# j-min/HiREST

Measured on AMD Instinct MI355X. Metric: encoded frames/sec (EVA-CLIP-g/14 224^2), higher is better.
Workload: dtype bf16

## Files before the change

hirest_amd/csrc/gemm.hip:

```cpp
#include <cstdio>
#include <atomic>
#include "gemm_shared.h"

namespace {


constexpr int BM = 128, BN = 128, BK = 64;
constexpr int STAGE_BYTES = (BM + BN) * BK * 2;

template <int EPI>
__device__ __forceinline__ void epilogue_store(const GemmP& p, int m, int n, f32x4 v) {
    if (p.bias) {
        f32x4 b = *reinterpret_cast<const f32x4*>(p.bias + n);
        v += b;
    }
    if constexpr (EPI == HIREST_EPI_BIAS_BF16 || EPI == HIREST_EPI_BIAS_GELU_BF16 || EPI == HIREST_EPI_BIAS_QGELU_BF16) {
        if constexpr (EPI == HIREST_EPI_BIAS_GELU_BF16) {
#pragma unroll
            for (int i = 0; i < 4; ++i) v[i] = gelu_erf(v[i]);
        }
        if constexpr (EPI == HIREST_EPI_BIAS_QGELU_BF16) {
#pragma unroll
            for (int i = 0; i < 4; ++i) v[i] = quick_gelu(v[i]);
        }
// ... 1000 lines not shown
    const int np_solo = team_walk && solo ? (np * solo + nslot / 2) / nslot : 0, np_team = np - np_solo;
    int count;
    if (!team_walk) count = (nunit - slot + nslot - 1) / nslot;
    else if (slot < tslots) { const int tm = slot / p.nbn; count = tm < np_team ? (np_team - tm + teams - 1) / teams : 0; }
    else { const int sl_ = slot - tslots; count = sl_ < np_solo ? ((np_solo - sl_ + solo - 1) / solo) * p.nbn : 0; }
    if (count <= 0) return;
    if (stagger) {
        const int who = stagger == 1 ? (slot & 3) : stagger == 2 ? (xcd & 3) : ((slot + xcd) & 7);
        const int units = who * (stagger == 3 ? (p.K / Q_BK + 15) / 16 : (p.K / Q_BK + 7) / 8);
        for (int i = 0; i < units; ++i) __builtin_amdgcn_s_sleep(127);
    }
    auto team_origin = [&](int i, int& M0, int& N0) {
        if (p.rev) i = count - 1 - i;
        int panel, col;
        if (slot < tslots) { panel = slot / p.nbn + i * teams; col = slot % p.nbn; }
        else { panel = np_team + (slot - tslots) + (i / p.nbn) * solo; col = i % p.nbn; }
        M0 = (p_lo + panel) * T_BM; N0 = col * T_BN;
    };
    auto tile_origin = [&](int j, int& M0, int& N0) {
        if (team_walk) { team_origin((j - slot) / nslot, M0, N0); return; }
        if (p.rev) j = nunit - 1 - j;
        if (panel_major) {
            const int mt_i = j / p.nbn;
            M0 = (p_lo + mt_i) * T_BM; N0 = (j - mt_i * p.nbn) * T_BN;
            return;
        }
        const int g_ = j / (GROUP_M * p.nbn);
        const int r = j - g_ * GROUP_M * p.nbn;
        int gcount = np - g_ * GROUP_M; gcount = gcount > GROUP_M ? GROUP_M : gcount;
        const int nt_i = r / gcount, mt_i = p_lo + g_ * GROUP_M + (r - nt_i * gcount);
        M0 = mt_i * T_BM; N0 = nt_i * T_BN;
    };

    const int nst = p.K / Q_BK;
    uint32_t a_off[2][2], w_off[2][2];
    int a_lds[2][2], w_lds[2][2];
    const char* a_base; const char* w_base;
#pragma unroll
    for (int hsel = 0; hsel < 2; ++hsel)
#pragma unroll
        for (int q = 0; q < 2; ++q) {
            const int j = 2 * wave + q;
            a_lds[hsel][q] = ((j >> 3) * 128 + hsel * 64 + (j & 7) * 8) * 128;
            w_lds[hsel][q] = Q_WOFF + ((j >> 2) * 64 + hsel * 32 + (j & 3) * 8) * 128;
        }
    auto set_sources = [&](int M0, int N0) {
#pragma unroll
        for (int hsel = 0; hsel < 2; ++hsel)
#pragma unroll
            for (int q = 0; q < 2; ++q) {
                const int ra0 = (a_lds[hsel][q] >> 7) + (lane >> 3);
                const int rw0 = ((w_lds[hsel][q] - Q_WOFF) >> 7) + (lane >> 3);
                const int ca = (lane & 7) ^ ((ra0 >> 1) & 7), cw = (lane & 7) ^ ((rw0 >> 1) & 7);
                int ra = p.M - 1 - M0; ra = ra0 < ra ? ra0 : ra;
                int rn = p.N - 1 - N0; rn = rw0 < rn ? rw0 : rn;
                a_off[hsel][q] = (uint32_t)(ra * (int)p.lda + ca * 8) * 2u;
                w_off[hsel][q] = (uint32_t)(rn * (int)p.ldw + cw * 8) * 2u;
            }
        const int Ma = (DBG && (sched & 8)) ? (p_lo + ((M0 / T_BM - p_lo) & 3)) * T_BM : M0;
        a_base = reinterpret_cast<const char*>(p.A + (int64_t)Ma * p.lda);
        w_base = reinterpret_cast<const char*>(p.W + (int64_t)N0 * p.ldw);
    };
    int dma_j = slot, dma_k = 0, dma_g = 0;
    bool dma_live = true;
    const char* a1_base; uint32_t a1_off[2]; int a1_k = 0, a1_g = 0;
    auto issue_a0 = [&]() {
        char* buf = smem + (dma_g & 1) * Q_STEP;
        const char* ab = a_base + (int64_t)dma_k * (Q_BK * 2);
        glds16(ab + a_off[0][0], buf + a_lds[0][0]);
        glds16(ab + a_off[0][1], buf + a_lds[0][1]);
    };
    auto issue_w = [&](int hsel) {
        char* buf = smem + (dma_g & 1) * Q_STEP;
        const char* wb = w_base + (int64_t)dma_k * (Q_BK * 2);
        glds16(wb + w_off[hsel][0], buf + w_lds[hsel][0]);
        glds16(wb + w_off[hsel][1], buf + w_lds[hsel][1]);
    };
    auto issue_a1_pending = [&]() {
        char* buf = smem + (a1_g & 1) * Q_STEP;
        const char* ab = a1_base + (int64_t)a1_k * (Q_BK * 2);
        glds16(ab + a1_off[0], buf + a_lds[1][0]);
        glds16(ab + a1_off[1], buf + a_lds[1][1]);
    };
    auto advance = [&]() {
        a1_base = a_base; a1_off[0] = a_off[1][0]; a1_off[1] = a_off[1][1]; a1_k = dma_k; a1_g = dma_g;
        ++dma_g;
        if (dma_live && ++dma_k == nst) {
            dma_j += nslot;
            if (dma_j < slot + count * nslot) { int m0, n0; tile_origin(dma_j, m0, n0); set_sources(m0, n0); dma_k = 0; }
            else { dma_live = false; dma_k = nst - 1; }
        }
    };

    const int frow = lane & 15, fsw = (frow >> 1) & 7, kg = lane >> 4;
    const int a_frag = (wr * 128 + frow) * (Q_BK * 2);
    const int w_frag = Q_WOFF + (wc * 64 + frow) * (Q_BK * 2);
    int koff[2];
#pragma unroll
    for (int h = 0; h < 2; ++h) koff[h] = ((4 * h + kg) ^ fsw) << 4;
    struct FA { bf16x8 v[4][2]; };
    struct FW { bf16x8 v[2][2]; };
    FA Af;
    FW W0, W1;
    auto read_a = [&](const char* buf, int a) {
#pragma unroll
        for (int m = 0; m < 4; ++m)
#pragma unroll
            for (int h = 0; h < 2; ++h) Af.v[m][h] = *reinterpret_cast<const bf16x8*>(buf + a_frag + (a * 64 + m * 16) * 128 + koff[h]);
    };
    auto read_w = [&](const char* buf, int b, FW& f) {
#pragma unroll
        for (int n = 0; n < 2; ++n)
#pragma unroll
            for (int h = 0; h < 2; ++h) f.v[n][h] = *reinterpret_cast<const bf16x8*>(buf + w_frag + (b * 32 + n * 16) * 128 + koff[h]);
    };
    f32x4 acc[8][NI];
    auto mfma_q = [&](int a, int b, FW& fw) {
        __builtin_amdgcn_s_setprio(1);
        if constexpr (X3) {
#pragma unroll
            for (int g3 = 0; g3 < 3; ++g3)
#pragma unroll
                for (int m = 0; m < 4; ++m)
#pragma unroll
                    for (int n = 0; n < 2; ++n)
                        acc[a * 4 + m][b * 2 + n] = __builtin_amdgcn_mfma_f32_16x16x32_bf16(fw.v[n][g3 == 1 ? 1 : 0], Af.v[m][g3 == 0 ? 1 : 0],
                                                                                             acc[a * 4 + m][b * 2 + n], 0, 0, 0);
        } else {
#pragma unroll
            for (int h = 0; h < 2; ++h)
#pragma unroll
                for (int m = 0; m < 4; ++m)
#pragma unroll
                    for (int n = 0; n < 2; ++n)
                        acc[a * 4 + m][b * 2 + n] = __builtin_amdgcn_mfma_f32_16x16x32_bf16(fw.v[n][h], Af.v[m][h], acc[a * 4 + m][b * 2 + n], 0, 0, 0);
        }
        __builtin_amdgcn_s_setprio(0);
    };
    auto bar = [&]() { __builtin_amdgcn_s_barrier(); };

    {
        int m0, n0;
        tile_origin(slot, m0, n0);
        set_sources(m0, n0);
    }
    for (int i = 0; i < 2; ++i) { issue_a0(); issue_w(0); issue_w(1); advance(); issue_a1_pending(); }
    bool a1_valid = false;
    HX_WAIT_VM(0);
    bar();
    if (grp == 1) bar();

    char* stg = smem + 2 * Q_STEP + wave * p_stg_bytes(EPI);
    int g = 0;
    for (int j = slot; j < slot + count * nslot; j += nslot) {
        int M0, N0;
        tile_origin(j, M0, N0);
        const bool active = (N0 + wc * 64 < p.N) && (M0 + wr * 128 < p.M);
        if (active) {
            if constexpr (epi_is_lnfold(EPI)) {
                int r0 = M0 + wr * 128 + 2 * lane;
                const int last = (p.M - 1) & ~1;
                r0 = r0 < last ? r0 : last;
                glds16(reinterpret_cast<const float*>(p.aux0) + 2 * (int64_t)r0, stg + P_STG);
                int c = N0 + wc * 64 + 4 * (lane & 15);
                c = c < p.N - 4 ? c : p.N - 4;
                const float* src = ((lane & 16) || !p.bias) ? reinterpret_cast<const float*>(p.aux1) : p.bias;
                glds16(src + c, stg + P_BCS);
            }
#pragma unroll
            for (int i = 0; i < 8; ++i)
#pragma unroll
                for (int jn = 0; jn < NI; ++jn) acc[i][jn] = f32x4{0.f, 0.f, 0.f, 0.f};
        }
        if (active && PH2) {
            for (int t = 0; t < nst; ++t, ++g) {
                const char* cur = smem + (g & 1) * Q_STEP;
                HX_WAIT_VM(6);
                __builtin_amdgcn_sched_barrier(0);
                read_a(cur, 0); read_w(cur, 0, W0); read_w(cur, 1, W1);
                if (a1_valid) issue_a1_pending();
                HX_WAIT_LGKM0();
                bar();
                mfma_q(0, 0, W0);
                mfma_q(0, 1, W1);
                bar();
                HX_WAIT_VM(2);
                __builtin_amdgcn_sched_barrier(0);
                read_a(cur, 1);
                issue_a0(); issue_w(0); issue_w(1);
                advance();
                a1_valid = true;
                HX_WAIT_LGKM0();
                bar();
                mfma_q(1, 1, W1);
                mfma_q(1, 0, W0);
                bar();
            }
            epilogue_p<EPI, NI, epi_is_lnfold(EPI), 8, RD, false, DBG, epi_is_lnfold(EPI)>(p, acc, stg, M0 + wr * 128, N0 + wc * 64, lane);
        } else if (PH2) {
            for (int t = 0; t < nst; ++t, ++g) {
                HX_WAIT_VM(6);
                if (a1_valid) issue_a1_pending();
                bar(); bar();
                HX_WAIT_VM(2);
                issue_a0(); issue_w(0); issue_w(1);
                advance();
                a1_valid = true;
                bar(); bar();
            }
        } else if (active) {
            for (int t = 0; t < nst; ++t, ++g) {
                const char* cur = smem + (g & 1) * Q_STEP;
                HX_WAIT_VM(8);
                __builtin_amdgcn_sched_barrier(0);
                read_a(cur, 0); read_w(cur, 0, W0);
                if (a1_valid) issue_a1_pending();
                bar();
                HX_WAIT_LGKM0();
                mfma_q(0, 0, W0);
                bar();
                HX_WAIT_VM(8);
                __builtin_amdgcn_sched_barrier(0);
                read_w(cur, 1, W1);
                bar();
                HX_WAIT_LGKM0();
                mfma_q(0, 1, W1);
                bar();
                __builtin_amdgcn_sched_barrier(0);
                read_a(cur, 1);
                issue_a0(); issue_w(0);
                bar();
                HX_WAIT_LGKM0();
                mfma_q(1, 1, W1);
                bar();
                HX_WAIT_VM(8);
                __builtin_amdgcn_sched_barrier(0);
                issue_w(1);
                advance();
                a1_valid = true;
                bar();
                mfma_q(1, 0, W0);
                bar();
            }
            if constexpr (epi_is_lnfold(EPI)) HX_WAIT_VM(8);
            epilogue_p<EPI, NI, epi_is_lnfold(EPI), 8, RD, false, DBG, epi_is_lnfold(EPI)>(p, acc, stg, M0 + wr * 128, N0 + wc * 64, lane);
        } else {
            for (int t = 0; t < nst; ++t, ++g) {
                HX_WAIT_VM(8);
                if (a1_valid) issue_a1_pending();
                bar(); bar();
                HX_WAIT_VM(8);
                bar(); bar();
                issue_a0(); issue_w(0);
                bar(); bar();
                HX_WAIT_VM(8);
                issue_w(1);
                advance();
                a1_valid = true;
                bar(); bar();
            }
        }
    }
    if (grp == 0) bar();
    HX_WAIT_VM(0);
}

template <int EPI, int RD = 1>
__global__ __launch_bounds__(512) void gemm_pp256(GemmP p) { pp256_body<EPI, RD, false>(p); }
template <int EPI>
__global__ __launch_bounds__(512) void gemm_pp256x3(GemmP p) { pp256_body<EPI, 1, true>(p); }
template <int EPI>
__global__ __launch_bounds__(512) void gemm_pq256(GemmP p) { pp256_body<EPI, (EPI == HIREST_EPI_BIAS_RESID2_LNSTATS ? HIREST_S2_RD : 1), false, 1>(p); }
template <int EPI>
__global__ __launch_bounds__(512) void gemm_pq256x3(GemmP p) { pp256_body<EPI, 1, true, 1>(p); }
template <int EPI>
__global__ __launch_bounds__(512) void gemm_pq256_dbg(GemmP p) { pp256_body<EPI, (EPI == HIREST_EPI_BIAS_RESID2_LNSTATS ? HIREST_S2_RD : 1), false, 1, true>(p); }



static inline void tiles256(GemmP& p) {
    p.nbm = (p.M + T_BM - 1) / T_BM; p.nbn = (p.N + T_BN - 1) / T_BN;
    p.ppx = (p.nbm + 7) / 8;
}

template <auto KERN, int LDS>
int launch_tiles(GemmP p, hipStream_t s) {
    static HirestDevCfg cfg;
    if (int e = hirest_configure(KERN, LDS, cfg)) return e;
    tiles256(p);
    hipLaunchKernelGGL(KERN, dim3(8 * p.ppx * p.nbn), dim3(512), LDS, s, p);
    return hirest_launch_status();
}
template <auto KERN, int NW, int LDS>
int launch_persistent(GemmP p, hipStream_t s) {
    static HirestDevCfg cfg;
    int cus = 0;
    if (int e = hirest_configure(KERN, LDS, cfg, &cus)) return e;
    tiles256(p);
    int nslot = cus / 8; nslot = nslot < 1 ? 1 : nslot;
    const int per_xcd = p.ppx * p.nbn;
    if (nslot > per_xcd) nslot = per_xcd;
    hipLaunchKernelGGL(KERN, dim3(8 * nslot), dim3(64 * NW), LDS, s, p);
    return hirest_launch_status();
}
constexpr int p_lds(int epi, int nw) { return 2 * Q_STEP + nw * p_stg_bytes(epi); }

template <int EPI>
int launch_t128(GemmP p, hipStream_t s) {
    hipLaunchKernelGGL(gemm_t128<EPI>, dim3(8 * p.ppx * p.nbn), dim3(256), 2 * STAGE_BYTES, s, p);
    return hirest_launch_status();
}

template <int EPI, int WM>
int launch_t128x3(GemmP p, hipStream_t s) {
    static HirestDevCfg cfg;
    auto kern = gemm_t128x3<EPI, WM>;
    constexpr int LDS = 4 * (64 * WM + BN) * BK * 2;
    if (int e = hirest_configure(kern, LDS, cfg)) return e;
    p.nbm = (p.M + 64 * WM - 1) / (64 * WM);
    p.ppx = (p.nbm + 7) / 8;
    p.flat = p.nbm < 32 ? 1 : 0;
    p.ksplit = 1;
    if (EPI == HIREST_EPI_BIAS_RESID_F32 && p.flat && p.aux0 && !p.aux1) {
        const int ntile = p.nbm * p.nbn, nk = p.K / BK;
        for (int S = 4; S >= 2; --S)
            if (nk % S == 0 && nk / S >= 8 && ntile * S <= 256) { p.ksplit = S; break; }
        p.part = reinterpret_cast<float*>(p.aux0);
    }
    const int grid = p.flat ? 8 * ((p.nbm * p.nbn * p.ksplit + 7) / 8) : 8 * p.ppx * p.nbn;
    hipLaunchKernelGGL(kern, dim3(grid), dim3(256 * WM), LDS, s, p);
    if (p.ksplit > 1) {
        const int64_t total = (int64_t)p.M * (p.N / 4);
        int blocks = (int)((total + 255) / 256); blocks = blocks > 2048 ? 2048 : blocks;
        hipLaunchKernelGGL(splitk_reduce_kernel, dim3(blocks), dim3(256), 0, s, p.part, p.ksplit, p.bias, reinterpret_cast<float*>(p.out), p.ldo, p.M, p.N);
    }
    return hirest_launch_status();
}

}
// ... 179 lines not shown
```

hirest_amd/csrc/gemm_shared.h:

```cpp
#pragma once
#include "common.h"
#include "profile.h"

namespace {

struct GemmP {
    const bf16_t* A; int64_t lda;
    const bf16_t* W; int64_t ldw;
    const float* bias;
    void* out; int64_t ldo;
    int M, N, K;
    const float* pos; int P;
    int rev;
    void* aux0; void* aux1;
    int nbm, nbn, ppx;
    int epi_dbg;
    int stagger;
    int sched;
    int dbg;
    int flat = 0;
    int ksplit = 1;
    float* part = nullptr;
};
constexpr int GEMM_DBG_IGNORE_REVERSE = 1 << 9;
constexpr int GEMM_DBG_STAGGER_SHIFT = 10, GEMM_DBG_STAGGER_MASK = 3;
constexpr int GEMM_DBG_EPI_SHIFT = 12, GEMM_DBG_EPI_MASK = 15;
constexpr int GEMM_DBG_SCHED_SHIFT = 16, GEMM_DBG_SCHED_MASK = 15;
constexpr int GEMM_DBG_PQ_SWITCHES = GEMM_DBG_STAGGER_MASK << GEMM_DBG_STAGGER_SHIFT | GEMM_DBG_EPI_MASK << GEMM_DBG_EPI_SHIFT | GEMM_DBG_SCHED_MASK << GEMM_DBG_SCHED_SHIFT;
constexpr int GEMM_DBG_KERNEL_BITS = ~(GEMM_DBG_IGNORE_REVERSE | GEMM_DBG_PQ_SWITCHES);

constexpr int GROUP_M = 8;
template <bool DBG = false>
__device__ __forceinline__ void xcd_panels(const GemmP& p, int xcd, int& p_lo, int& np) {
    if (DBG && (p.sched & 1)) { p_lo = xcd * p.ppx; np = p.nbm - p_lo; np = np > p.ppx ? p.ppx : np; return; }
    p_lo = (int)(((long long)xcd * p.nbm) >> 3);
    np = (int)(((long long)(xcd + 1) * p.nbm) >> 3) - p_lo;
}
constexpr int T_BM = 256, T_BN = 256;
#define HX_WAIT_VM(n) asm volatile("s_waitcnt vmcnt(" #n ")" ::: "memory")
#define HX_WAIT_LGKM0() asm volatile("s_waitcnt lgkmcnt(0)" ::: "memory")
constexpr int Q_BK = 64;
constexpr int Q_STEP = (T_BM + T_BN) * Q_BK * 2;
constexpr int Q_WOFF = T_BM * Q_BK * 2;

#ifndef HIREST_X3_GELU_POLY
#define HIREST_X3_GELU_POLY 1
#endif
#ifndef HIREST_S2_BUFFER_EPILOGUE
#define HIREST_S2_BUFFER_EPILOGUE 1
#endif
#ifndef HIREST_S2_RD
#define HIREST_S2_RD 2
#endif
constexpr int P_STG = 2048;
constexpr bool epi_is_lnfold(int epi) { return epi == HIREST_EPI_LNFOLD_BF16 || epi == HIREST_EPI_LNFOLD_GELU_BF16; }
constexpr int P_BCS = P_STG + 1024;
constexpr int p_stg_bytes(int epi) {
    return epi_is_lnfold(epi) ? P_STG + 2048 : (epi == HIREST_EPI_BIAS_RESID2_LNSTATS && HIREST_S2_BUFFER_EPILOGUE) ? 2 * P_STG : P_STG;
}

#define HX_LDS_ORDER() asm volatile("" ::: "memory")

__device__ __forceinline__ float dpp_xor1(float v) {
    return __builtin_bit_cast(float, __builtin_amdgcn_mov_dpp(__builtin_bit_cast(int, v), 0xB1, 0xf, 0xf, true));
}
__device__ __forceinline__ float sum8(float v) {
    v += __builtin_bit_cast(float, __builtin_amdgcn_mov_dpp(__builtin_bit_cast(int, v), 0xB1, 0xf, 0xf, true));
    v += __builtin_bit_cast(float, __builtin_amdgcn_mov_dpp(__builtin_bit_cast(int, v), 0x4E, 0xf, 0xf, true));
    v += __builtin_bit_cast(float, __builtin_amdgcn_mov_dpp(__builtin_bit_cast(int, v), 0x141, 0xf, 0xf, true));
    return v;
}
typedef __attribute__((ext_vector_type(4))) unsigned u32x4;
typedef __attribute__((ext_vector_type(2))) unsigned u32x2;
constexpr unsigned HX_OOB = 0x80000000u;
__device__ __forceinline__ __amdgpu_buffer_rsrc_t hx_rsrc(const void* base, unsigned bytes) {
    return __builtin_amdgcn_make_buffer_rsrc(const_cast<void*>(base), 0, (int)bytes, 0x00020000);
}

template <int NI, int NM, int RD, bool S2 = false, bool DBG = false>
__device__ __forceinline__ void epilogue_lnstats(const GemmP& p, f32x4 (&acc)[8][NI], int jc, char* stg, int Mw, int Nw, int lane) {
    const int epi_dbg = DBG ? p.epi_dbg : 0, sched = DBG ? p.sched : 0;
    const int srow = lane & 15, kg = lane >> 4, sw = lane & 7;
    const int rr = lane >> 3, rc = lane & 7;
    float* outp = reinterpret_cast<float*>(p.out);
    bf16_t* xb = reinterpret_cast<bf16_t*>(p.aux0);
    float* part = reinterpret_cast<float*>(p.aux1);
    const int G = (p.N + 63) >> 6;
    f32x4 bv[4];
#pragma unroll
    for (int n = 0; n < 4; ++n) {
        const int col = Nw + n * 16 + 4 * kg;
        bv[n] = (p.bias && col < p.N) ? *reinterpret_cast<const f32x4*>(p.bias + col) : f32x4{0.f, 0.f, 0.f, 0.f};
    }
    const int n0 = Nw + rc * 4, n1 = Nw + 32 + rc * 4;
    bf16_t* xlo = reinterpret_cast<bf16_t*>(p.out);
    auto load_res = [&](int mi, f32x4 (&o)[2][2]) {
#pragma unroll
        for (int it = 0; it < 2; ++it) {
            const int m = Mw + mi * 16 + it * 8 + rr;
            if constexpr (S2) {
                const int64_t mr = m < p.M ? m : p.M - 1;
                const int col = (rc & 1) ? n1 - 4 : n0;
                union { bf16x8 v; bf16x4 h[2]; float f[4]; } hv, lv;
                hv.v = bf16x8{0, 0, 0, 0, 0, 0, 0, 0}; lv.v = hv.v;
                if (col + 8 <= p.N && !(epi_dbg & 1)) {
                    if (sched & 2) {
                        hv.v = *reinterpret_cast<const bf16x8*>(xb + mr * p.N + col);
                        lv.v = *reinterpret_cast<const bf16x8*>(xlo + mr * p.ldo + col);
                    } else {
                        hv.v = __builtin_nontemporal_load(reinterpret_cast<const bf16x8*>(xb + mr * p.N + col));
                        lv.v = __builtin_nontemporal_load(reinterpret_cast<const bf16x8*>(xlo + mr * p.ldo + col));
                    }
                }
                o[0][it] = __builtin_bit_cast(f32x4, hv.v);
                o[1][it] = __builtin_bit_cast(f32x4, lv.v);
                continue;
            }
            const float* row = outp + (int64_t)(m < p.M ? m : p.M - 1) * p.ldo;
            o[0][it] = (n0 < p.N && !(epi_dbg & 1)) ? __builtin_nontemporal_load(reinterpret_cast<const f32x4*>(row + n0)) : f32x4{0.f, 0.f, 0.f, 0.f};
            o[1][it] = (n1 < p.N && !(epi_dbg & 1)) ? __builtin_nontemporal_load(reinterpret_cast<const f32x4*>(row + n1)) : f32x4{0.f, 0.f, 0.f, 0.f};
        }
    };
    f32x4 ring[RD + 1][2][2];
#pragma unroll
    for (int a = 0; a < RD && a < NM; ++a) load_res(a, ring[a]);
#pragma unroll
    for (int mi = 0; mi < NM; ++mi) {
        if (mi + RD < NM) load_res(mi + RD, ring[(mi + RD) % (RD + 1)]);
        f32x4 (&oc)[2][2] = ring[mi % (RD + 1)];
        if constexpr (S2) {
#pragma unroll
            for (int it = 0; it < 2; ++it) {
                union { bf16x8 v; bf16x4 h[2]; float f[4]; } hv, lv;
                hv.v = __builtin_bit_cast(bf16x8, oc[0][it]); lv.v = __builtin_bit_cast(bf16x8, oc[1][it]);
                union { bf16x4 v; float f[2]; } hs, hr, ls, lr;
                hs.v = (rc & 1) ? hv.h[0] : hv.h[1];
                ls.v = (rc & 1) ? lv.h[0] : lv.h[1];
                hr.f[0] = dpp_xor1(hs.f[0]); hr.f[1] = dpp_xor1(hs.f[1]);
                lr.f[0] = dpp_xor1(ls.f[0]); lr.f[1] = dpp_xor1(ls.f[1]);
                const bf16x4 h0 = (rc & 1) ? hr.v : hv.h[0], h1 = (rc & 1) ? hv.h[1] : hr.v;
                const bf16x4 l0 = (rc & 1) ? lr.v : lv.h[0], l1 = (rc & 1) ? lv.h[1] : lr.v;
#pragma unroll
                for (int e = 0; e < 4; ++e) { oc[0][it][e] = (float)h0[e] + (float)l0[e]; oc[1][it][e] = (float)h1[e] + (float)l1[e]; }
            }
        }
        f32x4 wv[2][2];
#pragma unroll
        for (int h = 0; h < 2; ++h) {
#pragma unroll
            for (int nn = 0; nn < 2; ++nn)
                *reinterpret_cast<f32x4*>(stg + srow * 128 + (((nn * 4 + kg) ^ sw) << 4)) = acc[mi][jc + h * 2 + nn] + bv[h * 2 + nn];
            HX_LDS_ORDER();
#pragma unroll
            for (int it = 0; it < 2; ++it) {
                const int r = it * 8 + rr;
                wv[h][it] = *reinterpret_cast<const f32x4*>(stg + r * 128 + ((rc ^ (r & 7)) << 4)) + oc[h][it];
            }
            HX_LDS_ORDER();
        }
#pragma unroll
        for (int it = 0; it < 2; ++it) {
            const int m = Mw + mi * 16 + it * 8 + rr;
            const bool okm = m < p.M, ok0 = okm && n0 < p.N, ok1 = okm && n1 < p.N;
            if constexpr (!S2) {
                if (ok0 && !(epi_dbg & 2)) __builtin_nontemporal_store(wv[0][it], reinterpret_cast<f32x4*>(outp + (int64_t)m * p.ldo + n0));
                if (ok1 && !(epi_dbg & 2)) __builtin_nontemporal_store(wv[1][it], reinterpret_cast<f32x4*>(outp + (int64_t)m * p.ldo + n1));
            }
            union { bf16x4 v; float f[2]; } b0, b1, snd, rcv;
            float ps = 0.f, pq = 0.f;
#pragma unroll
            for (int e = 0; e < 4; ++e) {
                b0.v[e] = (bf16_t)wv[0][it][e]; b1.v[e] = (bf16_t)wv[1][it][e];
                const float f0 = ok0 ? (float)b0.v[e] : 0.f, f1 = ok1 ? (float)b1.v[e] : 0.f;
                ps += f0 + f1; pq = fmaf(f0, f0, fmaf(f1, f1, pq));
            }
            snd.v = (rc & 1) ? b0.v : b1.v;
            rcv.f[0] = dpp_xor1(snd.f[0]); rcv.f[1] = dpp_xor1(snd.f[1]);
            union { bf16x8 v; float f[4]; } w8;
            int col;
            if (rc & 1) { w8.f[0] = rcv.f[0]; w8.f[1] = rcv.f[1]; w8.f[2] = b1.f[0]; w8.f[3] = b1.f[1]; col = n1 - 4; }
            else        { w8.f[0] = b0.f[0]; w8.f[1] = b0.f[1]; w8.f[2] = rcv.f[0]; w8.f[3] = rcv.f[1]; col = n0; }
            if (okm && col + 8 <= p.N && !(epi_dbg & 4)) __builtin_nontemporal_store(w8.v, reinterpret_cast<bf16x8*>(xb + (int64_t)m * p.N + col));
            if constexpr (S2) {
                union { bf16x4 v; float f[2]; } l0, l1, ls, lr;
#pragma unroll
                for (int e = 0; e < 4; ++e) {
                    l0.v[e] = (bf16_t)(wv[0][it][e] - (float)b0.v[e]);
                    l1.v[e] = (bf16_t)(wv[1][it][e] - (float)b1.v[e]);
                }
                ls.v = (rc & 1) ? l0.v : l1.v;
                lr.f[0] = dpp_xor1(ls.f[0]); lr.f[1] = dpp_xor1(ls.f[1]);
                union { bf16x8 v; float f[4]; } q8;
                if (rc & 1) { q8.f[0] = lr.f[0]; q8.f[1] = lr.f[1]; q8.f[2] = l1.f[0]; q8.f[3] = l1.f[1]; }
                else        { q8.f[0] = l0.f[0]; q8.f[1] = l0.f[1]; q8.f[2] = lr.f[0]; q8.f[3] = lr.f[1]; }
                if (okm && col + 8 <= p.N && !(epi_dbg & 2)) __builtin_nontemporal_store(q8.v, reinterpret_cast<bf16x8*>(xlo + (int64_t)m * p.ldo + col));
            }
            ps = sum8(ps); pq = sum8(pq);
            if (rc == 0 && okm && Nw < p.N && !(epi_dbg & 8)) *reinterpret_cast<f32x2*>(part + ((int64_t)m * G + (Nw >> 6)) * 2) = f32x2{ps, pq};
        }
    }
}


template <int NI, int NM, int RD, bool DBG = false>
__device__ __forceinline__ void epilogue_lnstats2(const GemmP& p, f32x4 (&acc)[8][NI], int jc, char* stg, int Mw, int Nw, int lane) {
    const int epi_dbg = DBG ? p.epi_dbg : 0, sched = DBG ? p.sched : 0;
    const int srow = lane & 15, kg = lane >> 4, sw = lane & 7;
    const int rr = lane >> 3, rc = lane & 7;
    const int G = (p.N + 63) >> 6;
    const int N = p.N, ldo = (int)p.ldo;
    int rows = p.M - Mw; rows = rows < NM * 16 ? rows : NM * 16;
    const __amdgpu_buffer_rsrc_t rs_hi = hx_rsrc(reinterpret_cast<const bf16_t*>(p.aux0) + (int64_t)Mw * N, (unsigned)rows * (unsigned)N * 2u);
    const __amdgpu_buffer_rsrc_t rs_lo = hx_rsrc(reinterpret_cast<const bf16_t*>(p.out) + (int64_t)Mw * ldo, ((unsigned)(rows - 1) * (unsigned)ldo + (unsigned)N) * 2u);
    const __amdgpu_buffer_rsrc_t rs_pt = hx_rsrc(reinterpret_cast<const float*>(p.aux1) + ((int64_t)Mw * G + (Nw >> 6)) * 2, ((unsigned)(rows - 1) * (unsigned)G + 1u) * 8u);
    const __amdgpu_buffer_rsrc_t rs_b = hx_rsrc(p.bias, p.bias ? (unsigned)N * 4u : 0u);
    const int n0 = Nw + rc * 4, n1 = Nw + 32 + rc * 4;
    const f32x4 bias0 = __builtin_bit_cast(f32x4, __builtin_amdgcn_raw_buffer_load_b128(rs_b, (unsigned)n0 * 4u, 0, 0));
    const f32x4 bias1 = __builtin_bit_cast(f32x4, __builtin_amdgcn_raw_buffer_load_b128(rs_b, (unsigned)n1 * 4u, 0, 0));
    const int col = (rc & 1) ? n1 - 4 : n0;
    const bool col_ok = col + 8 <= N;
    const unsigned vh0 = col_ok ? (unsigned)(rr * N + col) * 2u : HX_OOB, vl0 = col_ok ? (unsigned)(rr * ldo + col) * 2u : HX_OOB;
    const unsigned vp0 = (rc == 0 && Nw < N) ? (unsigned)(rr * G) * 8u : HX_OOB;
    const unsigned sh = 16u * (unsigned)N, sl = 16u * (unsigned)ldo, sp = 64u * (unsigned)G;
    const unsigned vh_ld = (epi_dbg & 1) ? HX_OOB : vh0, vl_ld = (epi_dbg & 1) ? HX_OOB : vl0;
    const unsigned vh_st = (epi_dbg & 4) ? HX_OOB : vh0, vl_st = (epi_dbg & 2) ? HX_OOB : vl0, vp_st = (epi_dbg & 8) ? HX_OOB : vp0;
    auto load_res = [&](int mi, u32x4 (&o)[2][2]) {
#pragma unroll
        for (int it = 0; it < 2; ++it) {
            const int k = mi * 2 + it;
            const bool okm = k * 8 + rr < rows;
            const unsigned vh = okm ? vh_ld : HX_OOB, vl = okm ? vl_ld : HX_OOB;
            if (DBG && (sched & 2)) {
                o[0][it] = __builtin_amdgcn_raw_buffer_load_b128(rs_hi, vh, (unsigned)k * sh, 0);
                o[1][it] = __builtin_amdgcn_raw_buffer_load_b128(rs_lo, vl, (unsigned)k * sl, 0);
            } else {
                o[0][it] = __builtin_amdgcn_raw_buffer_load_b128(rs_hi, vh, (unsigned)k * sh, 2);
                o[1][it] = __builtin_amdgcn_raw_buffer_load_b128(rs_lo, vl, (unsigned)k * sl, 2);
            }
        }
    };
    u32x4 ring[RD + 1][2][2];
#pragma unroll
    for (int a = 0; a < RD && a < NM; ++a) load_res(a, ring[a]);
#pragma unroll
    for (int mi = 0; mi < NM; ++mi) {
        if (mi + RD < NM) load_res(mi + RD, ring[(mi + RD) % (RD + 1)]);
        __builtin_amdgcn_sched_barrier(0);
#pragma unroll
        for (int h = 0; h < 2; ++h)
#pragma unroll
            for (int nn = 0; nn < 2; ++nn)
                *reinterpret_cast<f32x4*>(stg + h * P_STG + srow * 128 + (((nn * 4 + kg) ^ sw) << 4)) = acc[mi][jc + h * 2 + nn];
        HX_LDS_ORDER();
#pragma unroll
        for (int it = 0; it < 2; ++it) {
            const int k = mi * 2 + it;
            const int r = it * 8 + rr;
            f32x4 oc0, oc1;
            {
                union { bf16x8 v; bf16x4 h[2]; float f[4]; } hv, lv;
                hv.v = __builtin_bit_cast(bf16x8, ring[mi % (RD + 1)][0][it]); lv.v = __builtin_bit_cast(bf16x8, ring[mi % (RD + 1)][1][it]);
                union { bf16x4 v; float f[2]; } hs, hr, ls, lr;
                hs.v = (rc & 1) ? hv.h[0] : hv.h[1];
                ls.v = (rc & 1) ? lv.h[0] : lv.h[1];
                hr.f[0] = dpp_xor1(hs.f[0]); hr.f[1] = dpp_xor1(hs.f[1]);
                lr.f[0] = dpp_xor1(ls.f[0]); lr.f[1] = dpp_xor1(ls.f[1]);
                const bf16x4 h0 = (rc & 1) ? hr.v : hv.h[0], h1 = (rc & 1) ? hv.h[1] : hr.v;
                const bf16x4 l0 = (rc & 1) ? lr.v : lv.h[0], l1 = (rc & 1) ? lv.h[1] : lr.v;
#pragma unroll
                for (int e = 0; e < 4; ++e) { oc0[e] = (float)h0[e] + (float)l0[e]; oc1[e] = (float)h1[e] + (float)l1[e]; }
            }
            const f32x4 wv0 = (*reinterpret_cast<const f32x4*>(stg + r * 128 + ((rc ^ (r & 7)) << 4)) + bias0) + oc0;
            const f32x4 wv1 = (*reinterpret_cast<const f32x4*>(stg + P_STG + r * 128 + ((rc ^ (r & 7)) << 4)) + bias1) + oc1;
            const bool okm = k * 8 + rr < rows, ok0 = okm && n0 < N, ok1 = okm && n1 < N;
            union { bf16x4 v; float f[2]; } b0, b1, snd, rcv;
            float ps = 0.f, pq = 0.f;
#pragma unroll
            for (int e = 0; e < 4; ++e) {
                b0.v[e] = (bf16_t)wv0[e]; b1.v[e] = (bf16_t)wv1[e];
                const float f0 = ok0 ? (float)b0.v[e] : 0.f, f1 = ok1 ? (float)b1.v[e] : 0.f;
                ps += f0 + f1; pq = fmaf(f0, f0, fmaf(f1, f1, pq));
            }
            snd.v = (rc & 1) ? b0.v : b1.v;
            rcv.f[0] = dpp_xor1(snd.f[0]); rcv.f[1] = dpp_xor1(snd.f[1]);
            union { u32x4 u; float f[4]; } w8;
            if (rc & 1) { w8.f[0] = rcv.f[0]; w8.f[1] = rcv.f[1]; w8.f[2] = b1.f[0]; w8.f[3] = b1.f[1]; }
            else        { w8.f[0] = b0.f[0]; w8.f[1] = b0.f[1]; w8.f[2] = rcv.f[0]; w8.f[3] = rcv.f[1]; }
            __builtin_amdgcn_raw_buffer_store_b128(w8.u, rs_hi, okm ? vh_st + (unsigned)k * sh : HX_OOB, 0, 2);
            union { bf16x4 v; float f[2]; } l0, l1, ls, lr;
#pragma unroll
            for (int e = 0; e < 4; ++e) {
                l0.v[e] = (bf16_t)(wv0[e] - (float)b0.v[e]);
                l1.v[e] = (bf16_t)(wv1[e] - (float)b1.v[e]);
            }
            ls.v = (rc & 1) ? l0.v : l1.v;
            lr.f[0] = dpp_xor1(ls.f[0]); lr.f[1] = dpp_xor1(ls.f[1]);
            union { u32x4 u; float f[4]; } q8;
            if (rc & 1) { q8.f[0] = lr.f[0]; q8.f[1] = lr.f[1]; q8.f[2] = l1.f[0]; q8.f[3] = l1.f[1]; }
            else        { q8.f[0] = l0.f[0]; q8.f[1] = l0.f[1]; q8.f[2] = lr.f[0]; q8.f[3] = lr.f[1]; }
            __builtin_amdgcn_raw_buffer_store_b128(q8.u, rs_lo, okm ? vl_st + (unsigned)k * sl : HX_OOB, 0, 2);
            ps = sum8(ps); pq = sum8(pq);
            union { u32x2 u; float f[2]; } st;
            st.f[0] = ps; st.f[1] = pq;
            __builtin_amdgcn_raw_buffer_store_b64(st.u, rs_pt, okm ? vp_st + (unsigned)k * sp : HX_OOB, 0, 0);
        }
        HX_LDS_ORDER();
        __builtin_amdgcn_sched_barrier(0);
    }
}

__device__ __forceinline__ f32x4 load_row_stats(const GemmP& p, int Mw, int lane) {
    const float* st = reinterpret_cast<const float*>(p.aux0);
    const int r0 = Mw + 2 * lane;
    const f32x2 v0 = *reinterpret_cast<const f32x2*>(st + 2 * (int64_t)(r0 < p.M ? r0 : p.M - 1));
    const f32x2 v1 = *reinterpret_cast<const f32x2*>(st + 2 * (int64_t)(r0 + 1 < p.M ? r0 + 1 : p.M - 1));
    return f32x4{v0[0], v0[1], v1[0], v1[1]};
}

template <int EPI, int NI, bool PRE = false, int NM = 8, int RD = 1, bool SREG = false, bool DBG = false, bool BLDS = false>
__device__ __forceinline__ void epilogue_p(const GemmP& p, f32x4 (&acc)[8][NI], char* stg, int Mw, int Nw, int lane) {
    if constexpr (EPI == HIREST_EPI_BIAS_RESID_LNSTATS_F32 || EPI == HIREST_EPI_BIAS_RESID2_LNSTATS) {
#pragma unroll
        for (int jc = 0; jc < NI; jc += 4)
            if (Nw + jc * 16 < p.N) {
                if constexpr (EPI == HIREST_EPI_BIAS_RESID2_LNSTATS && HIREST_S2_BUFFER_EPILOGUE) epilogue_lnstats2<NI, NM, RD, DBG>(p, acc, jc, stg, Mw, Nw + jc * 16, lane);
                else epilogue_lnstats<NI, NM, RD, EPI == HIREST_EPI_BIAS_RESID2_LNSTATS, DBG>(p, acc, jc, stg, Mw, Nw + jc * 16, lane);
            }
        return;
    }
    constexpr bool FOLD = epi_is_lnfold(EPI);
    constexpr bool OUT_BF16 = (EPI == HIREST_EPI_BIAS_BF16 || EPI == HIREST_EPI_BIAS_GELU_BF16 || EPI == HIREST_EPI_BIAS_QGELU_BF16 || FOLD);
    const int srow = lane & 15, kg = lane >> 4, sw = lane & 7;
    const int rr = lane >> 3, rc = lane & 7;
    if constexpr (OUT_BF16) {
        bf16_t* outp = reinterpret_cast<bf16_t*>(p.out);
        f32x2 mrs[SREG ? NM : 1];
        if constexpr (FOLD && SREG) {
            const float* st = reinterpret_cast<const float*>(p.aux0);
#pragma unroll
            for (int mi = 0; mi < NM; ++mi) {
                const int r = Mw + mi * 16 + srow;
                mrs[mi] = *reinterpret_cast<const f32x2*>(st + 2 * (int64_t)(r < p.M ? r : p.M - 1));
            }
        } else if constexpr (FOLD) {
            if constexpr (!PRE) *reinterpret_cast<f32x4*>(stg + P_STG + 16 * lane) = load_row_stats(p, Mw, lane);
            HX_LDS_ORDER();
        }
#pragma unroll
        for (int jp = 0; jp < NI; jp += 4) {
            f32x4 bv[4], sv[FOLD ? 4 : 1];
#pragma unroll
            for (int n = 0; n < 4; ++n) {
                const int col = Nw + (jp + n) * 16 + 4 * kg;
                if constexpr (FOLD && BLDS) {
                    static_assert(!BLDS || NI == 4, "one 64-column group per wave");
                    const f32x4 b = *reinterpret_cast<const f32x4*>(stg + P_BCS + (n * 16 + 4 * kg) * 4);
                    bv[n] = p.bias ? b : f32x4{0.f, 0.f, 0.f, 0.f};
                    sv[n] = *reinterpret_cast<const f32x4*>(stg + P_BCS + 256 + (n * 16 + 4 * kg) * 4);
                } else {
                    bv[n] = (p.bias && col < p.N) ? *reinterpret_cast<const f32x4*>(p.bias + col) : f32x4{0.f, 0.f, 0.f, 0.f};
                    if constexpr (FOLD)
                        sv[n] = col < p.N ? *reinterpret_cast<const f32x4*>(reinterpret_cast<const float*>(p.aux1) + col) : f32x4{0.f, 0.f, 0.f, 0.f};
                }
            }
            f32x2 mr_next = {0.f, 1.f};
            if constexpr (FOLD && !SREG) mr_next = *reinterpret_cast<const f32x2*>(stg + P_STG + srow * 8);
#pragma unroll
            for (int mi = 0; mi < NM; ++mi) {
                f32x2 mr = mr_next;
                if constexpr (FOLD && SREG) mr = mrs[mi];
                if constexpr (FOLD && !SREG) { if (mi + 1 < NM) mr_next = *reinterpret_cast<const f32x2*>(stg + P_STG + ((mi + 1) * 16 + srow) * 8); }
#pragma unroll
                for (int n = 0; n < 4; ++n) {
                    f32x4 v;
                    if constexpr (FOLD) {
                        const float c = -mr[0] * mr[1];
                        v = acc[mi][jp + n] * f32x4{mr[1], mr[1], mr[1], mr[1]} + (sv[n] * f32x4{c, c, c, c} + bv[n]);
                    } else {
                        v = acc[mi][jp + n] + bv[n];
                    }
                    if constexpr (EPI == HIREST_EPI_BIAS_GELU_BF16 || EPI == HIREST_EPI_LNFOLD_GELU_BF16) {
                        const f32x2 g0 = gelu_erf2(f32x2{v[0], v[1]}), g1 = gelu_erf2(f32x2{v[2], v[3]});
                        v = f32x4{g0[0], g0[1], g1[0], g1[1]};
                    }
                    if constexpr (EPI == HIREST_EPI_BIAS_QGELU_BF16) {
#pragma unroll
                        for (int e = 0; e < 4; ++e) v[e] = quick_gelu(v[e]);
                    }
                    bf16x4 o;
#pragma unroll
                    for (int e = 0; e < 4; ++e) o[e] = (bf16_t)v[e];
                    *reinterpret_cast<bf16x4*>(stg + srow * 128 + (((n * 2 + (kg >> 1)) ^ sw) << 4) + (kg & 1) * 8) = o;
                }
                HX_LDS_ORDER();
                const int mb = Mw + mi * 16;
#pragma unroll
                for (int it = 0; it < 2; ++it) {
                    const int r = it * 8 + rr;
                    const bf16x8 v = *reinterpret_cast<const bf16x8*>(stg + r * 128 + ((rc ^ (r & 7)) << 4));
                    const int m = mb + r, n = Nw + jp * 16 + rc * 8;
                    if (m < p.M) {
                        bf16_t* dst = outp + (int64_t)m * p.ldo + n;
                        if (n + 8 <= p.N) __builtin_nontemporal_store(v, reinterpret_cast<bf16x8*>(dst));
                        else if (n + 4 <= p.N) *reinterpret_cast<bf16x4*>(dst) = bf16x4{v[0], v[1], v[2], v[3]};
                    }
                }
                HX_LDS_ORDER();
            }
        }
    } else if constexpr (EPI == HIREST_EPI_BIAS_GELU_SPLIT2) {
        bf16_t* outp = reinterpret_cast<bf16_t*>(p.out);
#pragma unroll
        for (int jp = 0; jp < NI; jp += 2) {
            if (Nw + jp * 16 >= p.N) continue;
            f32x4 bv[2];
#pragma unroll
            for (int n = 0; n < 2; ++n) {
                const int col = Nw + (jp + n) * 16 + 4 * kg;
                bv[n] = p.bias ? *reinterpret_cast<const f32x4*>(p.bias + col) : f32x4{0.f, 0.f, 0.f, 0.f};
            }
#pragma unroll
            for (int mi = 0; mi < NM; ++mi) {
#pragma unroll
                for (int n = 0; n < 2; ++n) {
                    const f32x4 v = acc[mi][jp + n] + bv[n];
                    bf16x4 hi, lo;
#if HIREST_X3_GELU_POLY
                    const f32x2 g0 = gelu_erf2(f32x2{v[0], v[1]}), g1 = gelu_erf2(f32x2{v[2], v[3]});
                    const f32x4 gv = {g0[0], g0[1], g1[0], g1[1]};
#else
                    f32x4 gv;
#pragma unroll
                    for (int e = 0; e < 4; ++e) gv[e] = 0.5f * v[e] * (1.0f + erff(v[e] * 0.70710678118654752440f));
#endif
#pragma unroll
                    for (int e = 0; e < 4; ++e) { hi[e] = (bf16_t)gv[e]; lo[e] = (bf16_t)(gv[e] - (float)hi[e]); }
                    *reinterpret_cast<bf16x4*>(stg + srow * 128 + (((n * 2 + (kg >> 1)) ^ sw) << 4) + (kg & 1) * 8) = hi;
                    *reinterpret_cast<bf16x4*>(stg + srow * 128 + (((4 + n * 2 + (kg >> 1)) ^ sw) << 4) + (kg & 1) * 8) = lo;
                }
                HX_LDS_ORDER();
                const int mb = Mw + mi * 16;
#pragma unroll
                for (int it = 0; it < 2; ++it) {
                    const int r = it * 8 + rr;
                    const bf16x8 v = *reinterpret_cast<const bf16x8*>(stg + r * 128 + ((rc ^ (r & 7)) << 4));
                    const int m = mb + r;
                    if (m < p.M) __builtin_nontemporal_store(v, reinterpret_cast<bf16x8*>(outp + (int64_t)m * p.ldo + 2 * (Nw + jp * 16) + rc * 8));
                }
                HX_LDS_ORDER();
            }
        }
    } else {
        float* outp = reinterpret_cast<float*>(p.out);
#pragma unroll
        for (int jp = 0; jp < NI; jp += 2) {
            f32x4 bv[2];
#pragma unroll
            for (int n = 0; n < 2; ++n) {
                const int col = Nw + (jp + n) * 16 + 4 * kg;
                bv[n] = (p.bias && col < p.N) ? *reinterpret_cast<const f32x4*>(p.bias + col) : f32x4{0.f, 0.f, 0.f, 0.f};
            }
            const int n = Nw + jp * 16 + rc * 4;
#pragma unroll
            for (int mh = 0; mh < NM; mh += 4) {
                f32x4 o[8];
#pragma unroll
                for (int it = 0; it < 8; ++it) {
                    const int m = Mw + mh * 16 + it * 8 + rr;
                    const bool ok = m < p.M && n < p.N;
                    if constexpr (EPI == HIREST_EPI_PATCH_POS_F32) {
                        const int mm = ok ? m : 0;
                        const int pp = mm % p.P;
                        o[it] = ok ? *reinterpret_cast<const f32x4*>(p.pos + (int64_t)(1 + pp) * p.N + n) : f32x4{0.f, 0.f, 0.f, 0.f};
                    } else if constexpr (EPI == HIREST_EPI_BIAS_RESID_F32) {
                        o[it] = ok ? __builtin_nontemporal_load(reinterpret_cast<const f32x4*>(outp + (int64_t)m * p.ldo + n)) : f32x4{0.f, 0.f, 0.f, 0.f};
                    }
                }
#pragma unroll
                for (int mi = mh; mi < mh + 4; ++mi) {
#pragma unroll
                    for (int nn = 0; nn < 2; ++nn) {
                        const f32x4 v = acc[mi][jp + nn] + bv[nn];
                        *reinterpret_cast<f32x4*>(stg + srow * 128 + (((nn * 4 + kg) ^ sw) << 4)) = v;
                    }
                    HX_LDS_ORDER();
#pragma unroll
                    for (int it = 0; it < 2; ++it) {
                        const int r = it * 8 + rr;
                        f32x4 w = *reinterpret_cast<const f32x4*>(stg + r * 128 + ((rc ^ (r & 7)) << 4));
                        if constexpr (EPI != HIREST_EPI_BIAS_F32) w += o[(mi - mh) * 2 + it];
                        const int m = Mw + mi * 16 + r;
                        if (m < p.M && n < p.N) {
                            int64_t off;
                            if constexpr (EPI == HIREST_EPI_PATCH_POS_F32) {
                                const int b = m / p.P, pp = m - b * p.P;
                                off = ((int64_t)b * (p.P + 1) + 1 + pp) * p.ldo + n;
                            } else {
                                off = (int64_t)m * p.ldo + n;
                            }
                            __builtin_nontemporal_store(w, reinterpret_cast<f32x4*>(outp + off));
                        }
                    }
                    HX_LDS_ORDER();
                }
            }
        }
    }
}

}
```

Baseline: 2112.

## Relax first-step vmcnt waits after epilogue and use buffer stores for bf16 output

The bf16 epilogue now writes through raw buffer stores with a bounded resource, so out-of-range rows and columns are dropped by hardware and no per-store branches are needed. This makes the number of outstanding vector-memory ops per tile predictable. The persistent GEMM loop then raises the vmcnt threshold on the first K-step after an active tile, so the next tile's prefetch waits do not also drain the previous epilogue's stores. Static asserts tie the counts to the epilogue structure, and a wrong count would break correctness.

```diff
diff --git a/hirest_amd/csrc/gemm.hip b/hirest_amd/csrc/gemm.hip
--- a/hirest_amd/csrc/gemm.hip
+++ b/hirest_amd/csrc/gemm.hip
@@ -1176,10 +1176,15 @@
 
     char* stg = smem + 2 * Q_STEP + wave * p_stg_bytes(EPI);
     int g = 0;
+    constexpr int TVM = (PH2 && !X3 && p_tile_start_counted(EPI)) ? p_tile_vm(EPI) : 0;
+    constexpr int VM_Q1 = 6 + TVM < 63 ? 6 + TVM : 63, VM_Q2 = 2 + TVM < 63 ? 2 + TVM : 63;
+    bool after_epi = false;
     for (int j = slot; j < slot + count * nslot; j += nslot) {
         int M0, N0;
         tile_origin(j, M0, N0);
         const bool active = (N0 + wc * 64 < p.N) && (M0 + wr * 128 < p.M);
+        const bool relaxed = TVM > 0 && after_epi && nst >= 2;
+        after_epi = active;
         if (active) {
             if constexpr (epi_is_lnfold(EPI)) {
                 int r0 = M0 + wr * 128 + 2 * lane;
@@ -1199,7 +1204,8 @@
         if (active && PH2) {
             for (int t = 0; t < nst; ++t, ++g) {
                 const char* cur = smem + (g & 1) * Q_STEP;
-                HX_WAIT_VM(6);
+                if (TVM > 0 && t == 0 && relaxed) HX_WAIT_VM_N(VM_Q1);
+                else HX_WAIT_VM(6);
                 __builtin_amdgcn_sched_barrier(0);
                 read_a(cur, 0); read_w(cur, 0, W0); read_w(cur, 1, W1);
                 if (a1_valid) issue_a1_pending();
@@ -1208,7 +1214,8 @@
                 mfma_q(0, 0, W0);
                 mfma_q(0, 1, W1);
                 bar();
-                HX_WAIT_VM(2);
+                if (TVM > 0 && t == 0 && relaxed) HX_WAIT_VM_N(VM_Q2);
+                else HX_WAIT_VM(2);
                 __builtin_amdgcn_sched_barrier(0);
                 read_a(cur, 1);
                 issue_a0(); issue_w(0); issue_w(1);
diff --git a/hirest_amd/csrc/gemm_shared.h b/hirest_amd/csrc/gemm_shared.h
--- a/hirest_amd/csrc/gemm_shared.h
+++ b/hirest_amd/csrc/gemm_shared.h
@@ -38,6 +38,7 @@
 }
 constexpr int T_BM = 256, T_BN = 256;
 #define HX_WAIT_VM(n) asm volatile("s_waitcnt vmcnt(" #n ")" ::: "memory")
+#define HX_WAIT_VM_N(n) asm volatile("s_waitcnt vmcnt(%0)" ::"n"(n) : "memory")
 #define HX_WAIT_LGKM0() asm volatile("s_waitcnt lgkmcnt(0)" ::: "memory")
 constexpr int Q_BK = 64;
 constexpr int Q_STEP = (T_BM + T_BN) * Q_BK * 2;
@@ -52,11 +53,27 @@
 #ifndef HIREST_S2_RD
 #define HIREST_S2_RD 2
 #endif
+#ifndef HIREST_TILE_START_WAITS
+#define HIREST_TILE_START_WAITS 1
+#endif
 constexpr int P_STG = 2048;
 constexpr bool epi_is_lnfold(int epi) { return epi == HIREST_EPI_LNFOLD_BF16 || epi == HIREST_EPI_LNFOLD_GELU_BF16; }
 constexpr int P_BCS = P_STG + 1024;
 constexpr int p_stg_bytes(int epi) {
     return epi_is_lnfold(epi) ? P_STG + 2048 : (epi == HIREST_EPI_BIAS_RESID2_LNSTATS && HIREST_S2_BUFFER_EPILOGUE) ? 2 * P_STG : P_STG;
+}
+
+constexpr int P_PASSES = 8;
+constexpr int P_BF16_SETS = 2;
+constexpr int P_TILE_START_PIECES = 2;
+constexpr int P_S2_BIAS_LOADS = 2, P_S2_SETS = 2, P_S2_SET_LOADS = 2, P_S2_SET_STORES = 3;
+constexpr bool p_tile_start_counted(int epi) {
+    return epi_is_lnfold(epi) ? (HIREST_TILE_START_WAITS & 2) != 0 : (HIREST_TILE_START_WAITS & 1) != 0;
+}
+constexpr int p_tile_vm(int epi) {
+    return epi_is_lnfold(epi) ? P_PASSES * P_BF16_SETS + P_TILE_START_PIECES
+         : (epi == HIREST_EPI_BIAS_RESID2_LNSTATS && HIREST_S2_BUFFER_EPILOGUE) ? P_S2_BIAS_LOADS + P_PASSES * P_S2_SETS * (P_S2_SET_LOADS + P_S2_SET_STORES)
+         : 0;
 }
 
 #define HX_LDS_ORDER() asm volatile("" ::: "memory")
@@ -204,6 +221,9 @@
 
 template <int NI, int NM, int RD, bool DBG = false>
 __device__ __forceinline__ void epilogue_lnstats2(const GemmP& p, f32x4 (&acc)[8][NI], int jc, char* stg, int Mw, int Nw, int lane) {
+    static_assert(NM != P_PASSES || p_tile_vm(HIREST_EPI_BIAS_RESID2_LNSTATS) == P_S2_BIAS_LOADS + NM * P_S2_SETS * (P_S2_SET_LOADS + P_S2_SET_STORES),
+                  "p_tile_vm() is stale: gemm_pq256's tile-start waits count this epilogue's loads and stores");
+    static_assert(P_S2_BIAS_LOADS == 2 && P_S2_SET_LOADS == 2 && P_S2_SET_STORES == 3, "bias0 | bias1; hi, lo; hi', lo', partials");
     const int epi_dbg = DBG ? p.epi_dbg : 0, sched = DBG ? p.sched : 0;
     const int srow = lane & 15, kg = lane >> 4, sw = lane & 7;
     const int rr = lane >> 3, rc = lane & 7;
@@ -226,7 +246,7 @@
     const unsigned vh_st = (epi_dbg & 4) ? HX_OOB : vh0, vl_st = (epi_dbg & 2) ? HX_OOB : vl0, vp_st = (epi_dbg & 8) ? HX_OOB : vp0;
     auto load_res = [&](int mi, u32x4 (&o)[2][2]) {
 #pragma unroll
-        for (int it = 0; it < 2; ++it) {
+        for (int it = 0; it < P_S2_SETS; ++it) {
             const int k = mi * 2 + it;
             const bool okm = k * 8 + rr < rows;
             const unsigned vh = okm ? vh_ld : HX_OOB, vl = okm ? vl_ld : HX_OOB;
@@ -253,7 +273,7 @@
                 *reinterpret_cast<f32x4*>(stg + h * P_STG + srow * 128 + (((nn * 4 + kg) ^ sw) << 4)) = acc[mi][jc + h * 2 + nn];
         HX_LDS_ORDER();
 #pragma unroll
-        for (int it = 0; it < 2; ++it) {
+        for (int it = 0; it < P_S2_SETS; ++it) {
             const int k = mi * 2 + it;
             const int r = it * 8 + rr;
             f32x4 oc0, oc1;
@@ -333,7 +353,12 @@
     const int srow = lane & 15, kg = lane >> 4, sw = lane & 7;
     const int rr = lane >> 3, rc = lane & 7;
     if constexpr (OUT_BF16) {
-        bf16_t* outp = reinterpret_cast<bf16_t*>(p.out);
+        static_assert(!(FOLD && BLDS && NM == P_PASSES) || p_tile_vm(EPI) == (NI / 4) * NM * P_BF16_SETS + P_TILE_START_PIECES,
+                      "p_tile_vm() is stale: gemm_pq256's tile-start waits count this epilogue's stores");
+        const int ldo = (int)p.ldo;
+        int rows = p.M - Mw; rows = rows < NM * 16 ? rows : NM * 16;
+        const __amdgpu_buffer_rsrc_t rs_out = hx_rsrc(reinterpret_cast<const bf16_t*>(p.out) + (int64_t)Mw * ldo,
+                                                      rows > 0 ? ((unsigned)(rows - 1) * (unsigned)ldo + (unsigned)p.N) * 2u : 0u);
         f32x2 mrs[SREG ? NM : 1];
         if constexpr (FOLD && SREG) {
             const float* st = reinterpret_cast<const float*>(p.aux0);
@@ -363,6 +388,11 @@
                         sv[n] = col < p.N ? *reinterpret_cast<const f32x4*>(reinterpret_cast<const float*>(p.aux1) + col) : f32x4{0.f, 0.f, 0.f, 0.f};
                 }
             }
+            const int nb = Nw + jp * 16, nc = nb + rc * 8, left = p.N - nb;
+            const unsigned s8 = 16u * (unsigned)ldo;
+            const unsigned v16 = nc + 8 <= p.N ? (unsigned)(rr * ldo + nc) * 2u : HX_OOB;
+            const bool edge4 = left > 0 && left < 64 && (left & 4);
+            const unsigned v8 = (nc + 8 > p.N && nc + 4 <= p.N) ? (unsigned)(rr * ldo + nc) * 2u : HX_OOB;
             f32x2 mr_next = {0.f, 1.f};
             if constexpr (FOLD && !SREG) mr_next = *reinterpret_cast<const f32x2*>(stg + P_STG + srow * 8);
 #pragma unroll
@@ -393,17 +423,14 @@
                     *reinterpret_cast<bf16x4*>(stg + srow * 128 + (((n * 2 + (kg >> 1)) ^ sw) << 4) + (kg & 1) * 8) = o;
                 }
                 HX_LDS_ORDER();
-                const int mb = Mw + mi * 16;
-#pragma unroll
-                for (int it = 0; it < 2; ++it) {
+#pragma unroll
+                for (int it = 0; it < P_BF16_SETS; ++it) {
                     const int r = it * 8 + rr;
-                    const bf16x8 v = *reinterpret_cast<const bf16x8*>(stg + r * 128 + ((rc ^ (r & 7)) << 4));
-                    const int m = mb + r, n = Nw + jp * 16 + rc * 8;
-                    if (m < p.M) {
-                        bf16_t* dst = outp + (int64_t)m * p.ldo + n;
-                        if (n + 8 <= p.N) __builtin_nontemporal_store(v, reinterpret_cast<bf16x8*>(dst));
-                        else if (n + 4 <= p.N) *reinterpret_cast<bf16x4*>(dst) = bf16x4{v[0], v[1], v[2], v[3]};
-                    }
+                    union { bf16x8 v; u32x4 u; u32x2 h[2]; } w;
+                    w.v = *reinterpret_cast<const bf16x8*>(stg + r * 128 + ((rc ^ (r & 7)) << 4));
+                    const unsigned step = (unsigned)(mi * 2 + it) * s8;
+                    __builtin_amdgcn_raw_buffer_store_b128(w.u, rs_out, v16 + step, 0, 2);
+                    if (edge4) __builtin_amdgcn_raw_buffer_store_b64(w.h[0], rs_out, v8 + step, 0, 0);
                 }
                 HX_LDS_ORDER();
             }
```

New measurement: 2130 (median of 6 runs). No clear change (+0.9%).

## Remap LN-stats epilogue lanes to eight contiguous columns per lane

Applied to the files above, without the earlier changes.

Adds a default-on alternative lane mapping for the residual-plus-LN-stats GEMM epilogue. Each lane now owns eight contiguous output columns, which removes the DPP xor exchange used to assemble 16-byte stores. Partial sum and sum-of-squares are reduced with permlane16_swap plus DPP and written as packed 32-bit values. The LDS staging swizzle and read addresses change to match. The intent is fewer cross-lane shuffles and cleaner vector stores, at the risk of LDS bank conflicts or a different stats layout that downstream consumers must agree with.

```diff
diff --git a/hirest_amd/csrc/gemm_shared.h b/hirest_amd/csrc/gemm_shared.h
--- a/hirest_amd/csrc/gemm_shared.h
+++ b/hirest_amd/csrc/gemm_shared.h
@@ -49,6 +49,9 @@
 #ifndef HIREST_S2_BUFFER_EPILOGUE
 #define HIREST_S2_BUFFER_EPILOGUE 1
 #endif
+#ifndef HIREST_S2_LANE8
+#define HIREST_S2_LANE8 1
+#endif
 #ifndef HIREST_S2_RD
 #define HIREST_S2_RD 2
 #endif
@@ -205,8 +208,7 @@
 template <int NI, int NM, int RD, bool DBG = false>
 __device__ __forceinline__ void epilogue_lnstats2(const GemmP& p, f32x4 (&acc)[8][NI], int jc, char* stg, int Mw, int Nw, int lane) {
     const int epi_dbg = DBG ? p.epi_dbg : 0, sched = DBG ? p.sched : 0;
-    const int srow = lane & 15, kg = lane >> 4, sw = lane & 7;
-    const int rr = lane >> 3, rc = lane & 7;
+    const int srow = lane & 15, kg = lane >> 4;
     const int G = (p.N + 63) >> 6;
     const int N = p.N, ldo = (int)p.ldo;
     int rows = p.M - Mw; rows = rows < NM * 16 ? rows : NM * 16;
@@ -214,6 +216,92 @@
     const __amdgpu_buffer_rsrc_t rs_lo = hx_rsrc(reinterpret_cast<const bf16_t*>(p.out) + (int64_t)Mw * ldo, ((unsigned)(rows - 1) * (unsigned)ldo + (unsigned)N) * 2u);
     const __amdgpu_buffer_rsrc_t rs_pt = hx_rsrc(reinterpret_cast<const float*>(p.aux1) + ((int64_t)Mw * G + (Nw >> 6)) * 2, ((unsigned)(rows - 1) * (unsigned)G + 1u) * 8u);
     const __amdgpu_buffer_rsrc_t rs_b = hx_rsrc(p.bias, p.bias ? (unsigned)N * 4u : 0u);
+#if HIREST_S2_LANE8
+    const int hf = kg & 1, j = lane & 3, rr = ((lane >> 2) & 3) | ((lane >> 5) << 2);
+    const int col = Nw + hf * 32 + j * 8;
+    const f32x4 bias0 = __builtin_bit_cast(f32x4, __builtin_amdgcn_raw_buffer_load_b128(rs_b, (unsigned)col * 4u, 0, 0));
+    const f32x4 bias1 = __builtin_bit_cast(f32x4, __builtin_amdgcn_raw_buffer_load_b128(rs_b, (unsigned)col * 4u + 16u, 0, 0));
+    const bool col_ok = col + 8 <= N;
+    const unsigned vh0 = col_ok ? (unsigned)(rr * N + col) * 2u : HX_OOB, vl0 = col_ok ? (unsigned)(rr * ldo + col) * 2u : HX_OOB;
+    const unsigned vp0 = (j == 0 && Nw < N) ? (unsigned)(rr * G) * 8u + (unsigned)hf * 4u : HX_OOB;
+    const unsigned sh = 16u * (unsigned)N, sl = 16u * (unsigned)ldo, sp = 64u * (unsigned)G;
+    const unsigned vh_ld = (epi_dbg & 1) ? HX_OOB : vh0, vl_ld = (epi_dbg & 1) ? HX_OOB : vl0;
+    const unsigned vh_st = (epi_dbg & 4) ? HX_OOB : vh0, vl_st = (epi_dbg & 2) ? HX_OOB : vl0, vp_st = (epi_dbg & 8) ? HX_OOB : vp0;
+    const auto sx = [](int r) { return ((r >> 1) & 1) | ((r & 1) << 1) | (r & 4); };
+    const int wr = srow * 128 + ((kg ^ sx(srow)) << 4);
+    const int rd = hf * P_STG + rr * 128 + (((2 * j) ^ sx(rr)) << 4);
+    const int rows_rr = rows - rr;
+    auto load_res = [&](int mi, u32x4 (&o)[2][2]) {
+#pragma unroll
+        for (int it = 0; it < 2; ++it) {
+            const int k = mi * 2 + it;
+            const bool okm = k * 8 < rows_rr;
+            const unsigned vh = okm ? vh_ld : HX_OOB, vl = okm ? vl_ld : HX_OOB;
+            if (DBG && (sched & 2)) {
+                o[0][it] = __builtin_amdgcn_raw_buffer_load_b128(rs_hi, vh, (unsigned)k * sh, 0);
+                o[1][it] = __builtin_amdgcn_raw_buffer_load_b128(rs_lo, vl, (unsigned)k * sl, 0);
+            } else {
+                o[0][it] = __builtin_amdgcn_raw_buffer_load_b128(rs_hi, vh, (unsigned)k * sh, 2);
+                o[1][it] = __builtin_amdgcn_raw_buffer_load_b128(rs_lo, vl, (unsigned)k * sl, 2);
+            }
+        }
+    };
+    u32x4 ring[RD + 1][2][2];
+#pragma unroll
+    for (int a = 0; a < RD && a < NM; ++a) load_res(a, ring[a]);
+#pragma unroll
+    for (int mi = 0; mi < NM; ++mi) {
+        if (mi + RD < NM) load_res(mi + RD, ring[(mi + RD) % (RD + 1)]);
+        __builtin_amdgcn_sched_barrier(0);
+#pragma unroll
+        for (int h = 0; h < 2; ++h)
+#pragma unroll
+            for (int nn = 0; nn < 2; ++nn)
+                *reinterpret_cast<f32x4*>(stg + h * P_STG + (wr ^ (nn * 64))) = acc[mi][jc + h * 2 + nn];
+        HX_LDS_ORDER();
+#pragma unroll
+        for (int it = 0; it < 2; ++it) {
+            const int k = mi * 2 + it;
+            union { bf16x8 v; u32x4 u; } hv, lv;
+            hv.u = ring[mi % (RD + 1)][0][it]; lv.u = ring[mi % (RD + 1)][1][it];
+            f32x4 oc0, oc1;
+#pragma unroll
+            for (int e = 0; e < 4; ++e) { oc0[e] = (float)hv.v[e] + (float)lv.v[e]; oc1[e] = (float)hv.v[4 + e] + (float)lv.v[4 + e]; }
+            const f32x4 wv0 = (*reinterpret_cast<const f32x4*>(stg + rd + it * 1024) + bias0) + oc0;
+            const f32x4 wv1 = (*reinterpret_cast<const f32x4*>(stg + (rd ^ 16) + it * 1024) + bias1) + oc1;
+            const bool okm = k * 8 < rows_rr;
+            union { bf16x8 v; u32x4 u; } b8, q8;
+#pragma unroll
+            for (int e = 0; e < 4; ++e) { b8.v[e] = (bf16_t)wv0[e]; b8.v[4 + e] = (bf16_t)wv1[e]; }
+            __builtin_amdgcn_raw_buffer_store_b128(b8.u, rs_hi, okm ? vh_st + (unsigned)k * sh : HX_OOB, 0, 2);
+#pragma unroll
+            for (int e = 0; e < 4; ++e) {
+                q8.v[e] = (bf16_t)(wv0[e] - (float)b8.v[e]);
+                q8.v[4 + e] = (bf16_t)(wv1[e] - (float)b8.v[4 + e]);
+            }
+            __builtin_amdgcn_raw_buffer_store_b128(q8.u, rs_lo, okm ? vl_st + (unsigned)k * sl : HX_OOB, 0, 2);
+            const bool ok = okm && col_ok;
+            const auto x0 = __builtin_amdgcn_permlane16_swap(ok ? b8.u[0] : 0u, ok ? b8.u[2] : 0u, false, false);
+            const auto x1 = __builtin_amdgcn_permlane16_swap(ok ? b8.u[1] : 0u, ok ? b8.u[3] : 0u, false, false);
+            union { bf16x4 v; unsigned u[2]; } q0, q1;
+            q0.u[0] = x0[0]; q0.u[1] = x1[0]; q1.u[0] = x0[1]; q1.u[1] = x1[1];
+            float ps = 0.f, pq = 0.f;
+#pragma unroll
+            for (int e = 0; e < 4; ++e) {
+                const float f0 = (float)q0.v[e], f1 = (float)q1.v[e];
+                ps += f0 + f1; pq = fmaf(f0, f0, fmaf(f1, f1, pq));
+            }
+            lane_swap16(ps, pq);
+            float v = ps + pq;
+            v += __builtin_bit_cast(float, __builtin_amdgcn_mov_dpp(__builtin_bit_cast(int, v), 0xB1, 0xf, 0xf, true));
+            v += __builtin_bit_cast(float, __builtin_amdgcn_mov_dpp(__builtin_bit_cast(int, v), 0x4E, 0xf, 0xf, true));
+            __builtin_amdgcn_raw_buffer_store_b32(__builtin_bit_cast(unsigned, v), rs_pt, okm ? vp_st + (unsigned)k * sp : HX_OOB, 0, 0);
+        }
+        HX_LDS_ORDER();
+        __builtin_amdgcn_sched_barrier(0);
+    }
+#else
+    const int sw = lane & 7, rr = lane >> 3, rc = lane & 7;
     const int n0 = Nw + rc * 4, n1 = Nw + 32 + rc * 4;
     const f32x4 bias0 = __builtin_bit_cast(f32x4, __builtin_amdgcn_raw_buffer_load_b128(rs_b, (unsigned)n0 * 4u, 0, 0));
     const f32x4 bias1 = __builtin_bit_cast(f32x4, __builtin_amdgcn_raw_buffer_load_b128(rs_b, (unsigned)n1 * 4u, 0, 0));
@@ -307,6 +395,7 @@
         HX_LDS_ORDER();
         __builtin_amdgcn_sched_barrier(0);
     }
+#endif
 }
 
 __device__ __forceinline__ f32x4 load_row_stats(const GemmP& p, int Mw, int lane) {
```

After: 2144 before, 2158 after (median of 6 runs). No clear change (+0.7%).
